# KuldeepChoksi/video-anomaly-detection

Hardware: AMD Instinct MI355X
Metric: frames/sec/GPU (256x256 autoencoder scoring) + AUROC parity vs reference (higher is better)
Workload: dtype f32; 1 GPU; configs[1]: image autoencoder scoring, batch 512 synthetic 256x256x3 frames per GPU; chunk=512, weights=deterministic synthetic state dict (Xavier scale, randomised BN), collective=none (1 GPU)

## Files before the change

include/vad_hip.h:

```cpp
#ifndef VAD_HIP_H
#define VAD_HIP_H
#include <stddef.h>
#ifdef __cplusplus
extern "C" {
#endif

#define VAD_ABI_VERSION 3
#define VAD_OK 0
#define VAD_ERR_ARG (-1)
#define VAD_ERR_HIP (-2)
#define VAD_ERR_WS (-3)

#define VAD_ACT_NONE 0
#define VAD_ACT_LEAKY 1
#define VAD_ACT_RELU 2

#define VAD_PREC_FP32 0
#define VAD_PREC_SPLIT 1
#define VAD_PREC_BF16 2
#define VAD_PREC_BF16S 3
#define VAD_PREC_WINO 4

int vad_abi_version(void);
const char* vad_last_error(void);
// ... 1 lines not shown

size_t vad_pack_conv3x3_floats(int cout, int cin);
int vad_pack_conv3x3(const float* w_oihw, const float* bias, const float* const* bn,
                     int cout, int cin, int precision, float* w_packed, float* bias_out);

size_t vad_pack_conv3x3_c3_floats(int cout);
int vad_pack_conv3x3_c3(const float* w_oihw, const float* bias, const float* const* bn,
                        int cout, float* w_packed, float* bias_out);

size_t vad_pack_convt2x2_floats(int cin, int cout);
int vad_pack_convt2x2(const float* w_iohw, const float* bias, const float* const* bn,
                      int cin, int cout, int precision, float* w_packed, float* bias_out);

size_t vad_pack_conv1x1_floats(int cout, int cin);
int vad_pack_conv1x1(const float* w_oihw, const float* bias, int cout, int cin,
                     float* w_packed, float* bias_out);


int vad_conv3x3_c3(const float* x_nchw, const float* w_packed, const float* bias, float* out_nhwc,
                   int n, int h, int w, int cout, int act, int pool, void* stream);

int vad_conv3x3_c3_fused(const float* x_nchw, const float* w0, const float* b0, const float* w1, const float* b1,
                         float* out_nhwc, int n, int h, int w, int precision, void* stream);

int vad_conv3x3(const float* in_nhwc, long long in_fs, const float* w_packed, const float* bias,
                float* out_nhwc, long long out_fs, int n, int h, int w, int cin, int cout,
                int act, int pool, int precision, void* stream);

size_t vad_pack_conv3x3_wino_floats(int cout, int cin);
int vad_pack_conv3x3_wino(const float* w_oihw, const float* bias, const float* const* bn, int cout, int cin,
                          float* w_packed, float* bias_out);
int vad_conv3x3_wino(const float* in_nhwc, long long in_fs, const float* w_packed, const float* bias,
                     float* out_nhwc, long long out_fs, int n, int h, int w, int cin, int cout,
                     int act, int pool, void* stream);
int vad_convlstm_step_wino(const float* x, long long x_fs, const float* h_prev, long long h_prev_fs, const float* c_prev,
                           const float* w_packed, const float* bias, float* h_out, long long h_out_fs, float* c_out,
                           float* z_ws, int n, int h, int w, int cin_x, int hid, void* stream);

int vad_convt2x2(const float* in_nhwc, long long in_fs, const float* w_packed, const float* bias,
                 float* out_nhwc, long long out_fs, int n, int h, int w, int cin, int cout,
                 int act, int precision, void* stream);

int vad_conv1x1(const float* in_nhwc, const float* w_packed, const float* bias, float* out_nhwc,
                long long npix, int cin, int cout, void* stream);

int vad_convlstm_step(const float* x, long long x_fs, const float* h_prev, long long h_prev_fs,
// ... 240 lines not shown
```

video-anomaly-detection_amd/csrc/conv_mfma.hip:

```cpp
#include <atomic>
#include <type_traits>
#include "vad_common.h"

enum { MODE_PLAIN = 0, MODE_POOL = 1, MODE_LSTM = 2 };

struct Conv3P {
    const float* in;  long long in_fs;  int cin_a;
    const float* in2; long long in2_fs;
    const float* w;   const float* bias;
    float* out;       long long out_fs;
    const float* c_prev; float* c_out;
    const float* zx; long long zx_fs;
    const float* w0; const float* b0;
    int xu8;
    int n, h, w_, cin, cout, hid;
    int tiles_x, tiles_y, cblocks;
    unsigned nblocks;
    unsigned long long* dbg;
    int stagger;
    float* stats;
};

#define MFMA32(a, b, c) __builtin_amdgcn_mfma_f32_32x32x2f32((a), (b), (c), 0, 0, 0)
#define VAD_KORDER(jj) (((jj) == 1) ? 2 : ((jj) == 2) ? 1 : (jj))
// ... 411 lines not shown
        else { if (act == VAD_ACT_LEAKY) GATE_LAUNCH(VAD_ACT_LEAKY, 0) else if (act == VAD_ACT_RELU) GATE_LAUNCH(VAD_ACT_RELU, 0) else GATE_LAUNCH(VAD_ACT_NONE, 0) }
#undef GATE_LAUNCH
        VAD_LAUNCH_CHECK();
        return VAD_OK;
    }
    if (cout % 64 == 0) {
        const long long px = (long long)n * ((wd + 15) / 16);
        const long long nb_thr = cout % 128 == 0 ? px * ((h + 7) / 8) * (cout / 128) : px * ((h + 15) / 16) * (cout / 64);
        if (nb_thr < vad_num_cus() && !with_stats) return pool ? L3(32, 1, 1, 2, 2, MODE_POOL) : L3(32, 1, 1, 2, 2, MODE_PLAIN);
    }
    if (cout % 128 == 0) {
        const long long nb8 = (long long)n * ((wd + 15) / 16) * ((h + 7) / 8) * (cout / 128);
        if (!pool && nb8 < 768) return L3(32, 1, 2, 2, 2, MODE_PLAIN);
        return pool ? L3(32, 2, 2, 2, 2, MODE_POOL) : L3(32, 2, 2, 2, 2, MODE_PLAIN);
    } else if (cout % 64 == 0) {
        if (kn.conv64) return pool ? L3(32, 2, 1, 2, 2, MODE_POOL) : L3(32, 2, 1, 2, 2, MODE_PLAIN);
        return pool ? L3(32, 2, 2, 4, 1, MODE_POOL) : L3(32, 2, 2, 4, 1, MODE_PLAIN);
    } else {
        return pool ? L3(32, 2, 1, 4, 1, MODE_POOL) : L3(32, 2, 1, 4, 1, MODE_PLAIN);
    }
#undef L3
}

extern "C" int vad_conv3x3_c3_fused(const float* x, const float* w0, const float* b0, const float* w1,
                                    const float* b1, float* out, int n, int h, int wd, int precision, void* stream) {
    return vad_conv3x3_c3_fused_fmt(x, VAD_X_F32_NCHW, w0, b0, w1, b1, out, n, h, wd, precision, stream);
}

int vad_conv3x3_c3_fused_fmt(const void* x, int fmt, const float* w0, const float* b0, const float* w1,
                             const float* b1, float* out, int n, int h, int wd, int precision, void* stream) {
    VAD_REQUIRE(x && w0 && b0 && w1 && b1 && out, "conv3x3_c3_fused: null pointer");
    VAD_REQUIRE(precision == VAD_PREC_FP32 || precision == VAD_PREC_SPLIT, "conv3x3_c3_fused: precision=%d must be VAD_PREC_FP32 (0) or VAD_PREC_SPLIT (1)", precision);
    const ConvKnobs kn;
    VAD_REQUIRE(fmt == VAD_X_F32_NCHW || (fmt == VAD_X_U8_NHWC && (kn.variant != 0 || precision == VAD_PREC_SPLIT)),
                "conv3x3_c3_fused: input format %d unsupported (uint8 input needs the persistent kernel)", fmt);
    VAD_REQUIRE(n > 0 && h > 0 && wd > 0 && h % 2 == 0 && wd % 2 == 0, "conv3x3_c3_fused: bad shape %dx%d", h, wd);
    Conv3P p{};
    p.in = (const float*)x; p.in_fs = (long long)3 * h * wd; p.cin_a = 32;
    p.w = w1; p.bias = b1; p.out = out; p.out_fs = (long long)(h / 2) * (wd / 2) * 32;
    p.w0 = w0; p.b0 = b0; p.xu8 = fmt == VAD_X_U8_NHWC;
    p.h = h; p.w_ = wd; p.cin = 32; p.cout = 32; p.hid = 0;
    constexpr int TH = 16;
    p.tiles_x = (wd + 15) / 16; p.tiles_y = (h + TH - 1) / TH; p.cblocks = 1;
    const long long nb = (long long)n * p.tiles_x * p.tiles_y;
    VAD_REQUIRE(nb < (1ll << 31), "conv3x3_c3_fused: grid too large");
    p.nblocks = (unsigned)nb;
    p.n = n;
    if (precision == VAD_PREC_SPLIT) {
        static std::atomic<unsigned> grid_cap1{0};
        unsigned cap = grid_cap1.load(std::memory_order_relaxed);
        if (!cap) grid_cap1 = cap = persistent_grid(conv3x3_mfma_pkernel<32, 2, 1, 4, 1, MODE_POOL, VAD_ACT_LEAKY, 1, 1>, ~0u);
        p.dbg = g_vad_dbg;
        hipLaunchKernelGGL((conv3x3_mfma_pkernel<32, 2, 1, 4, 1, MODE_POOL, VAD_ACT_LEAKY, 1, 1>), dim3(persistent_grid_for(p, cap)), dim3(256), 0,
                           (hipStream_t)stream, p);
    } else if (kn.variant == 0) {
        hipLaunchKernelGGL((conv3x3_mfma_kernel<32, 2, 1, 4, 1, MODE_POOL, VAD_ACT_LEAKY, 1>), dim3((unsigned)nb), dim3(256), 0,
                           (hipStream_t)stream, p);
    } else {
        static std::atomic<unsigned> grid_cap{0};
        unsigned cap = grid_cap.load(std::memory_order_relaxed);
        if (!cap) grid_cap = cap = persistent_grid(conv3x3_mfma_pkernel<32, 2, 1, 4, 1, MODE_POOL, VAD_ACT_LEAKY, 1>, ~0u);
        p.dbg = g_vad_dbg;
        hipLaunchKernelGGL((conv3x3_mfma_pkernel<32, 2, 1, 4, 1, MODE_POOL, VAD_ACT_LEAKY, 1>), dim3(persistent_grid_for(p, cap)), dim3(256), 0,
                           (hipStream_t)stream, p);
    }
    VAD_LAUNCH_CHECK();
    return VAD_OK;
}

bool vad_convlstm_gate_wins(int n, int h, int wd, int hid) { const ConvKnobs kn; return kn.variant != 0 && !kn.no_small && vad_gate_kernel_wins(n, h, wd, hid, kn) != 0; }

bool vad_convlstm_small_wins(int n, int h, int wd, int hid) {
    const long long nb_big = (long long)n * ((wd + 15) / 16) * ((h + 3) / 4) * (hid / 64);
    const int ncu = vad_num_cus();
    const long long m_big = (nb_big + ncu - 1) / ncu;
    const double cost_big = 2.0 * (double)(m_big / 2) + 1.107 * (double)(m_big % 2);
    const double cost_small = 1.178 * (double)nb_big / (double)ncu;
    return nb_big < ncu || cost_small < cost_big;
}

extern "C" int vad_convlstm_step(const float* x, long long x_fs, const float* h_prev, long long h_prev_fs, const float* c_prev,
                                 const float* w, const float* bias, float* h_out, long long h_out_fs,
                                 float* c_out, int n, int h, int wd, int cin_x, int hid, int precision, void* stream) {
    return vad_convlstm_step_zx(x, x_fs, nullptr, 0, h_prev, h_prev_fs, c_prev, w, bias, h_out, h_out_fs, c_out, n, h, wd, cin_x, hid, precision, stream);
}

int vad_convlstm_step_zx(const float* x, long long x_fs, const float* zx, long long zx_fs, const float* h_prev, long long h_prev_fs,
// ... 742 lines not shown
```

video-anomaly-detection_amd/csrc/conv_pkernel.h:

```cpp
#pragma once

__device__ __forceinline__ void pf_set(float& d, float v) { d = v; }
__device__ __forceinline__ void pf_set(float& d, f32x4 v) { d = v[0]; }
__device__ __forceinline__ void pf_set(f32x4& d, f32x4 v) { d = v; }
__device__ __forceinline__ void pf_set(f32x4& d, float v) { d = f32x4{v, v, v, v}; }
__device__ __forceinline__ float pf_get_f(float v) { return v; }
__device__ __forceinline__ float pf_get_f(f32x4 v) { return v[0]; }
__device__ __forceinline__ f32x4 pf_get_v(f32x4 v) { return v; }
__device__ __forceinline__ f32x4 pf_get_v(float v) { return f32x4{v, v, v, v}; }
__device__ __forceinline__ void pf_set(u32x2& d, u32x2 v) { d = v; }
__device__ __forceinline__ void pf_set(u32x2& d, float) {}
__device__ __forceinline__ void pf_set(u32x2& d, f32x4) {}
__device__ __forceinline__ void pf_set(float& d, u32x2) {}
__device__ __forceinline__ void pf_set(f32x4& d, u32x2) {}
__device__ __forceinline__ float pf_get_f(u32x2 v) { return __uint_as_float(v[0]); }
__device__ __forceinline__ f32x4 pf_get_v(u32x2 v) { return f32x4{__uint_as_float(v[0]), __uint_as_float(v[1]), 0.f, 0.f}; }
__device__ __forceinline__ u32x2 pf_get_u(u32x2 v) { return v; }
__device__ __forceinline__ u32x2 pf_get_u(float) { return u32x2{0u, 0u}; }
__device__ __forceinline__ u32x2 pf_get_u(f32x4) { return u32x2{0u, 0u}; }

#ifdef VAD_STAMPS
#define STAMP(k)                                                                                      \
    {                                                                                                 \
        __builtin_amdgcn_sched_barrier(0);                                                            \
// ... 32 lines not shown
__device__ __forceinline__ void vad_mma16(f32x16& acc, f32x16& corr, f16x8 ah, f16x8 al, f16x8 bh, f16x8 bl) {
    if constexpr (PREC == 2) {
        acc = MFMAB16(ah, bh, acc);
    } else {
        acc = MFMA16(ah, bh, acc);
        corr = MFMA16(ah, bl, corr);
        corr = MFMA16(al, bh, corr);
    }
}

template <int PREC>
__device__ __forceinline__ void tile_put_t(float* tile, int pixoff_plus_ch, int ch, float v) {
    if constexpr (PREC) {
        _Float16 hi, lo;
        vad_split_p<PREC>(v, hi, lo);
        _Float16* blk = (_Float16*)&tile[pixoff_plus_ch - ch + (ch >> 3) * 8];
        blk[ch & 7] = hi;
        blk[8 + (ch & 7)] = lo;
    } else {
        tile[pixoff_plus_ch] = v;
    }
}

template <int CK, int MT, int NT, int WM, int WN, int MODE, int ACT, int FUSE_C3 = 0, int PREC = 0, int WITH_STATS = 0, int IO16 = 0>
__global__ __launch_bounds__(256, (FUSE_C3 && !PREC) ? 3 : 2) void conv3x3_mfma_pkernel(Conv3P p) {
    static_assert(WM * WN == 4, "4 waves per work-group");
    static_assert(MODE != MODE_LSTM || NT == 4, "LSTM mode: one N-tile per gate");
    static_assert(!FUSE_C3 || CK == 32, "fused first layer produces exactly one 32-channel chunk");
    static_assert(CK == 32, "staging slots assume 8 channel quads per pixel");
    static_assert(!IO16 || (PREC == 2 && MODE == MODE_PLAIN && !FUSE_C3), "bf16 tensors: bf16 operands, plain convolution");
    constexpr unsigned ES = IO16 ? 2u : 4u;
    constexpr int TH = 2 * MT * WM, LH = TH + 2, LW = 18, PS = CK + 4;
    constexpr int XH = LH + 2, XW = 20, XS = 20;
    constexpr int NPIX = LH * LW, NT0 = (NPIX + 31) / 32;
    constexpr int TOT = FUSE_C3 ? 3 * XH * XW : NPIX * (CK / 4), NPF = (TOT + 255) / 256;
    constexpr int KS = PREC ? 16 : 8;
    constexpr int NS = 9 * (CK / KS);
    constexpr int PB32 = (MODE == MODE_POOL || FUSE_C3) ? 1 : 3;
    constexpr int PB = (PREC == 2) ? 5 : (PREC && NT <= 2) ? 2 : PREC ? 1 : PB32, NB = PB + 1;
    static_assert(NS % 2 == 0 && NS % NB == 0, "fragment ring parity must be the same in every chunk");
    __shared__ __attribute__((aligned(16))) float tile[NPIX * PS];
    __shared__ float xin[FUSE_C3 ? 3 * XH * XS : 1];

    const int tid = threadIdx.x, lane = tid & 63, wave = tid >> 6;
    const int wm = wave / WN, wn = wave % WN;
    const int li = lane & 31, lh = lane >> 5;
    const int prow = (li >> 1) & 1, pcol = 2 * (li >> 2) + (li & 1);

    const unsigned per_frame = (unsigned)(p.tiles_x * p.tiles_y * p.cblocks);
    unsigned L = vad_xcd_remap(blockIdx.x % per_frame, per_frame);
    const int fg = blockIdx.x / per_frame, fgroups = gridDim.x / per_frame;
    const int cb = L % p.cblocks; L /= p.cblocks;
    constexpr bool STATS = WITH_STATS && MODE == MODE_PLAIN && ACT == VAD_ACT_NONE && !FUSE_C3;
    const unsigned stats_row = (unsigned)(blockIdx.x / per_frame) * (unsigned)(p.tiles_x * p.tiles_y) + L;
    float st_s[STATS ? NT : 1], st_q[STATS ? NT : 1];
#pragma unroll
    for (int nt = 0; nt < (STATS ? NT : 1); ++nt) st_s[nt] = st_q[nt] = 0.f;
    const int x0 = (L % p.tiles_x) * 16, y0 = (L / p.tiles_x) * TH;
    const int H = p.h, W = p.w_;

    int abase[MT];
#pragma unroll
    for (int mt = 0; mt < MT; ++mt)
        abase[mt] = ((2 * (wm * MT + mt) + prow) * LW + pcol) * PS + (PREC ? 8 : 4) * lh;

    const int nch_a = p.cin_a / CK;
    const int nch = (p.in2 ? p.cin : p.cin_a) / CK;
    const unsigned wstep = (unsigned)p.cout * (PREC ? 64u : 32u);
    const unsigned wtap = (unsigned)(p.cin / KS) * wstep;
    const __amdgpu_buffer_rsrc_t rw = vad_rsrc(p.w, (p.stagger & 1) ? 0u : 9u * wtap);

    unsigned svo[NPF];
    int slds0;
    const int c4 = tid & 7;
    if (FUSE_C3) {
        slds0 = 0;
#pragma unroll
        for (int i = 0; i < NPF; ++i) {
            const int idx = tid + 256 * i;
            const int lx = idx % XW, t = idx / XW, ly = t % XH, c = t / XH;
            const int gy = y0 - 2 + ly, gx = x0 - 2 + lx;
            const bool ok = idx < TOT && gy >= 0 && gy < H && gx >= 0 && gx < W;
            svo[i] = !ok ? VAD_OOB
                         : p.xu8 ? (unsigned)(__mul24(__mul24(gy, W) + gx, 3) + c)
                                 : (unsigned)(__mul24(c, __mul24(H, W)) + __mul24(gy, W) + gx) * 4u;
        }
    } else {
        const int pix0 = tid >> 3;
        slds0 = pix0 * PS + c4 * 4;
#pragma unroll
        for (int i = 0; i < NPF; ++i) {
            const int pix = pix0 + 32 * i;
            const int ly = pix / LW, lx = pix - ly * LW;
            const int gy = y0 - 1 + ly, gx = x0 - 1 + lx;
            const bool ok = pix < NPIX && gy >= 0 && gy < H && gx >= 0 && gx < W;
            svo[i] = ok ? (unsigned)(__mul24(__mul24(gy, W) + gx, p.cin_a) + c4 * 4) * ES : VAD_OOB;
        }
    }

    typedef typename std::conditional<FUSE_C3 != 0, float, typename std::conditional<IO16 != 0, u32x2, f32x4>::type>::type pf_t;
    pf_t pf[NPF];
    pf_t pf2[IO16 ? NPF : 1];
    float cpv[MODE == MODE_LSTM ? MT : 1][16];

    const unsigned in_bytes = FUSE_C3 ? (unsigned)(3 * H * W) * (p.xu8 ? 1u : 4u) : (unsigned)(H * W) * (unsigned)p.cin_a * ES;
#define ISSUE_TO(PF_, n_, ch_)         \
    {                                                                                                    \
        const char* src_ = ((ch_) < nch_a) ? (const char*)p.in + ((size_t)(n_) * p.in_fs + (ch_) * CK) * ES            \
                                           : (const char*)p.in2 + ((size_t)(n_) * p.in2_fs + ((ch_) - nch_a) * CK) * ES; \
        const unsigned skip_ = (unsigned)(((ch_) < nch_a) ? (ch_) : (ch_) - nch_a) * CK * ES;            \
        const __amdgpu_buffer_rsrc_t r_ = vad_rsrc(src_, in_bytes - skip_);                              \
        _Pragma("unroll") for (int i_ = 0; i_ < NPF; ++i_) {                                             \
            if constexpr (IO16) pf_set(PF_[i_], __builtin_bit_cast(u32x2, vad_bload2(r_, svo[i_], 0)));  \
            else pf_set(PF_[i_], vad_bload4(r_, svo[i_], 0));                                            \
        }                                                                                                \
    }
#define ISSUE(n_, ch_)                                                                                   \
    {                                                                                                    \
        if constexpr (FUSE_C3) {                                                                         \
            if (p.xu8) {    \
                const __amdgpu_buffer_rsrc_t r_ = vad_rsrc((const unsigned char*)p.in + (size_t)(n_) * p.in_fs, in_bytes); \
                _Pragma("unroll") for (int i_ = 0; i_ < NPF; ++i_)                                       \
                    pf_set(pf[i_], __uint_as_float((unsigned)(unsigned char)__builtin_amdgcn_raw_buffer_load_b8(r_, (int)svo[i_], 0, 0))); \
            } else {                                                                                     \
                const __amdgpu_buffer_rsrc_t r_ = vad_rsrc(p.in + (size_t)(n_) * p.in_fs, in_bytes);     \
                _Pragma("unroll") for (int i_ = 0; i_ < NPF; ++i_) pf_set(pf[i_], vad_bload1(r_, svo[i_], 0)); \
            }                                                                                            \
        } else {                                                                                         \
            const char* src_ = ((ch_) < nch_a) ? (const char*)p.in + ((size_t)(n_) * p.in_fs + (ch_) * CK) * ES            \
                                               : (const char*)p.in2 + ((size_t)(n_) * p.in2_fs + ((ch_) - nch_a) * CK) * ES; \
            const unsigned skip_ = (unsigned)(((ch_) < nch_a) ? (ch_) : (ch_) - nch_a) * CK * ES;        \
            const __amdgpu_buffer_rsrc_t r_ = vad_rsrc(src_, in_bytes - skip_);                          \
            _Pragma("unroll") for (int i_ = 0; i_ < NPF; ++i_) {                                         \
                if constexpr (IO16) pf_set(pf[i_], __builtin_bit_cast(u32x2, vad_bload2(r_, svo[i_], 0))); \
                else pf_set(pf[i_], vad_bload4(r_, svo[i_], 0));                                         \
            }                                                                                            \
        }                                                                                                \
    }

#define XWRITE(xb_)                                                                                      \
    {                                                                                                    \
        _Pragma("unroll") for (int i_ = 0; i_ < NPF; ++i_) {                                             \
            const int idx_ = tid + 256 * i_;                                                             \
            const int lx_ = idx_ % XW, t_ = idx_ / XW;                              \
            float xv_ = pf_get_f(pf[i_]);                                                                \
            if (p.xu8) xv_ = svo[i_] == VAD_OOB ? 0.f : vad_norm_u8(__float_as_uint(xv_));               \
            if (idx_ < TOT) (xb_)[t_ * XS + lx_] = xv_;                                                  \
        }                                                                                                \
    }

#ifdef VAD_STAMPS
    unsigned long long st_sum[10] = {0, 0, 0, 0, 0, 0, 0, 0, 0, 0}, st_prev = 0, st_n = 0;
    const unsigned long long st_t0 = __builtin_amdgcn_s_memtime(), st_r0 = __builtin_amdgcn_s_memrealtime();
#endif

    int n = fg;
    if (n >= p.n) return;
    ISSUE(n, 0);
    const bool deep = IO16 && nch >= 2 && (nch & 1) == 0;
    if constexpr (IO16) {
        if (deep) { ISSUE_TO(pf2, n, 1); }
    }
    if constexpr (FUSE_C3) {
        XWRITE(xin);
        if (n + fgroups < p.n) { ISSUE(n + fgroups, 0); }
    }

    f32x4 a[2][MT], b[NB][NT];
    f16x8 ah[PREC ? 1 : 2][MT], al[PREC ? 1 : 2][MT], bh[NB][NT], bl[NB][NT];
    unsigned wl[NT];
// ... 24 lines not shown
        _Pragma("unroll") for (int mt = (m0); mt < (m1); ++mt) {                                  \
            ah[0][mt] = __builtin_bit_cast(f16x8, *(const f32x4*)&tile[abase[mt] + toff_]);       \
            al[0][mt] = __builtin_bit_cast(f16x8, *(const f32x4*)&tile[abase[mt] + toff_ + 4]);   \
        }                                                                                         \
    }
#define LOAD_A(buf, step)                                                                         \
    {                                                                                             \
        const int toff_ = ((((step) / (CK / KS)) / 3) * LW + (((step) / (CK / KS)) % 3)) * PS +   \
                          ((step) % (CK / KS)) * (PREC ? 16 : 8);                                 \
        _Pragma("unroll") for (int mt = 0; mt < MT; ++mt) {                                       \
            if constexpr (PREC) {                                                                 \
                ah[buf][mt] = __builtin_bit_cast(f16x8, *(const f32x4*)&tile[abase[mt] + toff_]); \
                al[buf][mt] = __builtin_bit_cast(f16x8, *(const f32x4*)&tile[abase[mt] + toff_ + 4]); \
            } else a[buf][mt] = *(const f32x4*)&tile[abase[mt] + toff_];                          \
        }                                                                                         \
    }
#pragma unroll
    for (int s0 = 0; s0 < PB; ++s0) LOAD_B(s0, 0, s0);

    float b0w[(FUSE_C3 && !PREC) ? 14 : 1];
    f16x8 b0h[(FUSE_C3 && PREC) ? 2 : 1], b0l[(FUSE_C3 && PREC) ? 2 : 1];
    float bias0 = 0.f;
    bool interior = false;
    if constexpr (FUSE_C3) {
        if constexpr (PREC) {
            const f32x4* ws = (const f32x4*)(p.w0 + 28 * 32);
#pragma unroll
            for (int ks = 0; ks < 2; ++ks) {
                b0h[ks] = __builtin_bit_cast(f16x8, ws[((ks * 32 + li) * 2 + lh) * 2]);
                b0l[ks] = __builtin_bit_cast(f16x8, ws[((ks * 32 + li) * 2 + lh) * 2 + 1]);
            }
        } else {
        }
        bias0 = p.b0[li];
        interior = y0 > 0 && x0 > 0 && y0 + TH < H && x0 + 16 < W;
    }
#pragma unroll
    for (int nt = 0; nt < NT; ++nt) asm volatile("" ::"v"(bv[nt]));
    if constexpr (FUSE_C3) {
        if constexpr (PREC) {
#pragma unroll
            for (int ks = 0; ks < 2; ++ks) { asm volatile("" ::"v"(b0h[ks])); asm volatile("" ::"v"(b0l[ks])); }
        }
        asm volatile("" ::"v"(bias0));
    }

    const bool full_tile = (y0 + TH <= H) && (x0 + 16 <= W);
    const int ech = (MODE == MODE_LSTM) ? p.hid : p.cout;
    const int ow = (MODE == MODE_POOL) ? (W >> 1) : W, oh = (MODE == MODE_POOL) ? (H >> 1) : H;
    const int ey0 = (MODE == MODE_POOL) ? (y0 >> 1) + wm * MT : y0 + 2 * wm * MT;
    const int ex0 = (MODE == MODE_POOL) ? (x0 >> 1) + lh : x0 + 2 * lh;
    const unsigned erow = (unsigned)__mul24(ow, ech) * ES, ecol = (unsigned)ech * ES;
    unsigned eoff[NT];
#pragma unroll
    for (int nt = 0; nt < NT; ++nt) eoff[nt] = (unsigned)(__mul24(__mul24(ey0, ow) + ex0, ech) + cofs[nt]) * ES;
    const unsigned out_bytes = (unsigned)__mul24(oh, ow) * (unsigned)ech * ES;

    while (true) {
        f32x16 acc[MT][NT];
        f32x16 corr[PREC == 1 ? MT : 1][PREC == 1 ? NT : 1];
        if constexpr (PREC == 1) {
#pragma unroll
            for (int mt = 0; mt < MT; ++mt)
#pragma unroll
                for (int nt = 0; nt < NT; ++nt)
#pragma unroll
                    for (int r = 0; r < 16; ++r) corr[mt][nt][r] = 0.f;
        }
        if constexpr (!FUSE_C3) {
#pragma unroll
            for (int mt = 0; mt < MT; ++mt)
#pragma unroll
                for (int nt = 0; nt < NT; ++nt)
#pragma unroll
                    for (int r = 0; r < 16; ++r) acc[mt][nt][r] = bv[nt];
// ... 82 lines not shown
#pragma unroll
                        for (int ks = 0; ks < 2; ++ks) {
                            c0 = MFMA16(gh[ks], b0h[ks], c0);
                            cc = MFMA16(gh[ks], b0l[ks], cc);
                            cc = MFMA16(gl[ks], b0h[ks], cc);
                        }
                        __builtin_amdgcn_s_setprio(0);
                        const int qb = (t * 32 + 4 * lh) * PS + li;
#pragma unroll
                        for (int r = 0; r < 16; ++r) {
                            const int q2 = t * 32 + (r & 3) + 8 * (r >> 2) + 4 * lh;
                            const int ly2 = q2 / LW, lx2 = q2 - ly2 * LW;
                            const bool inside = interior || ((unsigned)(y0 - 1 + ly2) < (unsigned)H && (unsigned)(x0 - 1 + lx2) < (unsigned)W);
                            const float v = vad_act(fmaf(cc[r], 0x1p-11f, c0[r]), VAD_ACT_LEAKY);
                            if (q2 < NPIX) tile_put_t<PREC>(tile, qb + ((r & 3) + 8 * (r >> 2)) * PS, li, inside ? v : 0.f);
                        }
                    }
                } else {
                constexpr int TPW = (NT0 + 3) / 4;
                f32x16 c0[TPW];
                f32x16 bias16;
#pragma unroll
                for (int r = 0; r < 16; ++r) bias16[r] = bias0;
                int abase0[TPW];
#pragma unroll
                for (int u = 0; u < TPW; ++u) {
                    const int q = (wave + 4 * u) * 32 + li, qc = q < NPIX ? q : NPIX - 1;
                    abase0[u] = (qc / LW) * XS + (qc % LW);
                }
#pragma unroll
                for (int h0 = 0; h0 < 14; h0 += 7) {
                    float av[TPW][7];
#pragma unroll
                    for (int u = 0; u < TPW; ++u)
#pragma unroll
                        for (int s0 = 0; s0 < 7; ++s0) {
                            const int k0 = 2 * (h0 + s0), k1 = 2 * (h0 + s0) + 1;
                            const int o0 = ((k0 / 9) * XH + (k0 % 9) / 3) * XS + (k0 % 3);
                            const int o1 = (k1 < 27) ? ((k1 / 9) * XH + (k1 % 9) / 3) * XS + (k1 % 3) : 0;
                            av[u][s0] = xin[abase0[u] + (lh ? o1 : o0)];
                        }
                    __builtin_amdgcn_sched_barrier(0);
                    __builtin_amdgcn_s_setprio(1);
#pragma unroll
                    for (int s0 = 0; s0 < 7; ++s0)
#pragma unroll
                        for (int u = 0; u < TPW; ++u) c0[u] = MFMA32(av[u][s0], b0w[h0 + s0], (h0 + s0 == 0) ? bias16 : c0[u]);
                    __builtin_amdgcn_s_setprio(0);
                    __builtin_amdgcn_sched_barrier(0);
                }
#pragma unroll
                for (int u = 0; u < TPW; ++u) {
                    const int t = wave + 4 * u;
                    if (t < NT0) {
                        const int qb = (t * 32 + 4 * lh) * PS + li;
                        if (interior && t < NT0 - 1) {
#pragma unroll
                            for (int r = 0; r < 16; ++r)
                                tile_put_t<PREC>(tile, qb + ((r & 3) + 8 * (r >> 2)) * PS, li, vad_act(c0[u][r], VAD_ACT_LEAKY));
                        } else {
#pragma unroll
                            for (int r = 0; r < 16; ++r) {
                                const int q2 = t * 32 + (r & 3) + 8 * (r >> 2) + 4 * lh;
                                const int ly2 = q2 / LW, lx2 = q2 - ly2 * LW;
                                const bool inside = (unsigned)(y0 - 1 + ly2) < (unsigned)H && (unsigned)(x0 - 1 + lx2) < (unsigned)W;
                                const float v = vad_act(c0[u][r], VAD_ACT_LEAKY);
                                if (q2 < NPIX) tile_put_t<PREC>(tile, qb + ((r & 3) + 8 * (r >> 2)) * PS, li, inside ? v : 0.f);
                            }
                        }
                    }
                }
                }
                STAMP(8);
                __syncthreads();
                STAMP(9);
                if (has_next) { XWRITE(xin); }
                if (nn + fgroups < p.n) { ISSUE(nn + fgroups, 0); }
#pragma unroll
                for (int mt = 0; mt < MT; ++mt)
#pragma unroll
                    for (int nt = 0; nt < NT; ++nt)
#pragma unroll
                        for (int r = 0; r < 16; ++r) acc[mt][nt][r] = bv[nt];
            } else {
#pragma unroll
                for (int i = 0; i < NPF; ++i)
                    if ((tid >> 3) + 32 * i < NPIX) {
                        if constexpr (IO16) {
                            float* blk = &tile[(tid >> 3) * PS + i * 32 * PS + (c4 >> 1) * 8 + (c4 & 1) * 2];
                            *(u32x2*)blk = pf_get_u(pf[i]);
                        } else if constexpr (PREC) {
                            const f32x4 v = pf_get_v(pf[i]);
                            float* blk = &tile[(tid >> 3) * PS + i * 32 * PS + (c4 >> 1) * 8 + (c4 & 1) * 2];
                            if constexpr (PREC == 2) {
                                typedef __bf16 bf16x2_t __attribute__((ext_vector_type(2)));
                                typedef unsigned u32x2_t __attribute__((ext_vector_type(2)));
                                const bf16x2_t p0 = {(__bf16)v[0], (__bf16)v[1]}, p1 = {(__bf16)v[2], (__bf16)v[3]};
                                *(u32x2_t*)blk = u32x2_t{__builtin_bit_cast(unsigned, p0), __builtin_bit_cast(unsigned, p1)};
                            } else {
                                f16x4 hi, lo;
#pragma unroll
                                for (int e = 0; e < 4; ++e) { _Float16 h_, l_; vad_split_p<PREC>(v[e], h_, l_); hi[e] = h_; lo[e] = l_; }
                                *(f16x4*)blk = hi;
                                *(f16x4*)(blk + 4) = lo;
                            }
                        } else {
// ... 80 lines not shown
#pragma unroll
            for (int s0 = 0; s0 < PB; ++s0) LOAD_B(s0, 0, s0);
        }

        if (MODE == MODE_LSTM) {
            const __amdgpu_buffer_rsrc_t rc_out = vad_rsrc(p.c_out + (size_t)n * (out_bytes / 4), out_bytes);
            const __amdgpu_buffer_rsrc_t rh_out = vad_rsrc(p.out + (size_t)n * p.out_fs, out_bytes);
#pragma unroll
            for (int mt = 0; mt < MT; ++mt) {
#pragma unroll
                for (int r = 0; r < 16; ++r) {
                    const int dy = 2 * mt + ((r & 3) >> 1), dx = 4 * (r >> 2) + (r & 1);
                    const bool ok = full_tile || ((ey0 + dy) < oh && (ex0 + dx) < ow);
                    const unsigned vo = ok ? eoff[0] : VAD_OOB;
                    const unsigned so = dy * erow + dx * ecol;
                    float cn, hn;
                    vad_lstm_cell(acc[mt][0][r], acc[mt][1][r], acc[mt][2][r], acc[mt][3][r], cpv[mt][r], cn, hn);
                    vad_bstore1(cn, rc_out, vo, so);
                    vad_bstore1(hn, rh_out, vo, so);
                }
            }
        } else {
            const __amdgpu_buffer_rsrc_t ro = vad_rsrc((const char*)p.out + (size_t)n * p.out_fs * ES, (p.stagger & 2) ? 0u : out_bytes);
            if (MODE == MODE_POOL) {
#pragma unroll
                for (int mt = 0; mt < MT; ++mt) {
#pragma unroll
                    for (int q = 0; q < 4; ++q) {
                        const bool ok = full_tile || ((ey0 + mt) < oh && (ex0 + 2 * q) < ow);
                        const unsigned so = mt * erow + 2 * q * ecol;
#pragma unroll
                        for (int nt = 0; nt < NT; ++nt) {
                            const float m = fmaxf(fmaxf(acc[mt][nt][4 * q], acc[mt][nt][4 * q + 1]), fmaxf(acc[mt][nt][4 * q + 2], acc[mt][nt][4 * q + 3]));
                            vad_bstore1(vad_act(m, ACT), ro, ok ? eoff[nt] : VAD_OOB, so);
                        }
                    }
                }
            } else {
                float ts[STATS ? NT : 1], tq[STATS ? NT : 1];
#pragma unroll
                for (int nt = 0; nt < (STATS ? NT : 1); ++nt) ts[nt] = tq[nt] = 0.f;
#pragma unroll
                for (int mt = 0; mt < MT; ++mt) {
#pragma unroll
                    for (int q = 0; q < 4; ++q) {
#pragma unroll
                        for (int pos = 0; pos < 4; ++pos) {
                            const int dy = 2 * mt + (pos >> 1), dx = 4 * q + (pos & 1);
                            const bool ok = full_tile || ((ey0 + dy) < oh && (ex0 + dx) < ow);
                            const unsigned so = dy * erow + dx * ecol;
#pragma unroll
                            for (int nt = 0; nt < NT; ++nt) {
// ... 63 lines not shown
```

video-anomaly-detection_amd/hip.py:

```python
from __future__ import annotations

import ctypes as C
import os
import subprocess
import threading
from pathlib import Path

PKG_DIR = Path(__file__).resolve().parent
REPO_DIR = PKG_DIR.parent
CSRC = PKG_DIR / "csrc"
LIB_PATH = Path(os.environ.get("VAD_LIB", PKG_DIR / "libvad_hip.so"))
SOURCES = ["conv_mfma.hip", "conv_wino.hip", "dec4_fused.hip", "tail.hip", "wide_io.hip", "state_io.hip", "resize_u8.hip", "ssim.hip", "train_ops.hip", "train_step.hip", "train_step_img.hip", "vad_api.hip", "pack.cpp"]

VAD_OK = 0
ABI_VERSION = 3
MAX_IN_CHANNELS = 32
PREC_FP32, PREC_SPLIT, PREC_BF16, PREC_BF16S, PREC_WINO = 0, 1, 2, 3, 4
PRECISIONS = {"fp32": PREC_FP32, "split": PREC_SPLIT, "bf16": PREC_BF16S, "bf16_operands": PREC_BF16, "bf16_tensors": PREC_BF16S,
              "winograd": PREC_WINO}


def training_precision(name: str, trainer: str, tensors: bool) -> str:
    ok = ("fp32", "split", "bf16_operands", "winograd") + (("bf16", "bf16_tensors") if tensors else ())
    if name in ("bf16", "bf16_tensors") and not tensors:
# ... 58 lines not shown

_f32p = C.POINTER(C.c_float)
_vp = C.c_void_p
_ll = C.c_longlong
_i = C.c_int
_sz = C.c_size_t
_f = C.c_float

SIGNATURES = {
    "vad_abi_version": (_i, []),
    "vad_last_error": (C.c_char_p, []),
    "vad_pack_conv3x3_floats": (_sz, [_i, _i]),
    "vad_pack_conv3x3": (_i, [_vp, _vp, _vp, _i, _i, _i, _vp, _vp]),
    "vad_pack_conv3x3_c3_floats": (_sz, [_i]),
    "vad_pack_conv3x3_c3": (_i, [_vp, _vp, _vp, _i, _vp, _vp]),
    "vad_pack_convt2x2_floats": (_sz, [_i, _i]),
    "vad_pack_convt2x2": (_i, [_vp, _vp, _vp, _i, _i, _i, _vp, _vp]),
    "vad_pack_conv1x1_floats": (_sz, [_i, _i]),
    "vad_pack_conv1x1": (_i, [_vp, _vp, _i, _i, _vp, _vp]),
    "vad_pack_conv3x3_to3_floats": (_sz, [_i]),
    "vad_pack_conv3x3_to3": (_i, [_vp, _i, _vp]),
    "vad_conv3x3_c3": (_i, [_vp, _vp, _vp, _vp, _i, _i, _i, _i, _i, _i, _vp]),
    "vad_conv3x3_c3_fused": (_i, [_vp, _vp, _vp, _vp, _vp, _vp, _i, _i, _i, _i, _vp]),
    "vad_conv3x3": (_i, [_vp, _ll, _vp, _vp, _vp, _ll, _i, _i, _i, _i, _i, _i, _i, _i, _vp]),
    "vad_convt2x2": (_i, [_vp, _ll, _vp, _vp, _vp, _ll, _i, _i, _i, _i, _i, _i, _i, _vp]),
    "vad_pack_conv3x3_wino_floats": (_sz, [_i, _i]),
    "vad_pack_conv3x3_wino": (_i, [_vp, _vp, _vp, _i, _i, _vp, _vp]),
    "vad_conv3x3_wino": (_i, [_vp, _ll, _vp, _vp, _vp, _ll, _i, _i, _i, _i, _i, _i, _i, _vp]),
    "vad_convlstm_step_wino": (_i, [_vp, _ll, _vp, _ll, _vp, _vp, _vp, _vp, _ll, _vp, _vp, _i, _i, _i, _i, _i, _vp]),
    "vad_conv1x1": (_i, [_vp, _vp, _vp, _vp, _ll, _i, _i, _vp]),
    "vad_convlstm_step": (_i, [_vp, _ll, _vp, _ll, _vp, _vp, _vp, _vp, _ll, _vp, _i, _i, _i, _i, _i, _i, _vp]),
    "vad_score_partials": (_i, [_i, _i, _i]),
    "vad_conv3x3_to3_score": (_i, [_vp, _vp, _vp, _vp, _vp, _vp, _vp, _i, _i, _i, _i, _vp]),
    "vad_convt2x2_to3_score": (_i, [_vp, _vp, _vp, _vp, _vp, _vp, _vp, _i, _i, _i, _i, _i, _i, _vp]),
    "vad_score_finalize": (_i, [_vp, _i, _i, _i, _i, _vp, _vp, _i, _vp]),
    "vad_nhwc_to_nchw": (_i, [_vp, _vp, _i, _i, _i, _i, _vp]),
    "vad_nchw_to_nhwc": (_i, [_vp, _vp, _i, _i, _i, _i, _vp]),
    "vad_ssim_workspace_floats": (_sz, [_ll, _i, _i]),
    "vad_ssim_mse": (_i, [_vp, _vp, _ll, _i, _i, _i, C.c_float, _vp, _vp, _vp]),
    "vad_ssim_grad_workspace_floats": (_sz, [_ll, _i, _i]),
    "vad_ssim_mse_backward": (_i, [_vp, _vp, _ll, _i, _i, _i, C.c_float, _vp, _vp, _vp, _vp]),
    "vad_chan_ws_floats": (_sz, [_ll, _i]),
    "vad_bn_stats": (_i, [_vp, _ll, _i, _f, _f, _vp, _vp, _vp, _vp, _vp]),
    "vad_chan_sum": (_i, [_vp, _ll, _i, _vp, _vp, _vp]),
    "vad_bn_act_pool_fwd": (_i, [_vp, _vp, _vp, _vp, _vp, _ll, _i, _i, _i, _i, _i, _i, _i, _i, _i, _vp]),
    "vad_bn_act_pool_bwd": (_i, [_vp, _vp, _vp, _vp, _vp, _ll, _i, _i, _i, _vp, _i, _vp, _vp, _vp, _vp,
# ... 195 lines not shown
```

Measured before the change: 17150 frames/s.

## Specialize fused first-layer persistent kernel on uint8 input and simplify halo handling

Adds a compile-time XU8 template parameter so the fused first conv layer branches on uint8-versus-float input at compile time instead of at runtime. In the fp32 path, per-element boundary checks on the layer-0 tile writes are replaced by a separate pass that zeroes only the out-of-image halo rows and columns of edge tiles. It also precomputes LDS address bases per tap delta, and adds a branch-free pooling epilogue for full tiles. This aims to cut ALU and branch overhead in the first layer, at the cost of an extra barrier on edge tiles and more kernel instantiations.

```diff
diff --git a/include/vad_hip.h b/include/vad_hip.h
--- a/include/vad_hip.h
+++ b/include/vad_hip.h
@@ -47,6 +47,8 @@
 
 int vad_conv3x3_c3_fused(const float* x_nchw, const float* w0, const float* b0, const float* w1, const float* b1,
                          float* out_nhwc, int n, int h, int w, int precision, void* stream);
+int vad_conv3x3_c3_fused_x(const void* x, int x_format, const float* w0, const float* b0, const float* w1, const float* b1,
+                           float* out_nhwc, int n, int h, int w, int precision, void* stream);
 
 int vad_conv3x3(const float* in_nhwc, long long in_fs, const float* w_packed, const float* bias,
                 float* out_nhwc, long long out_fs, int n, int h, int w, int cin, int cout,
diff --git a/video-anomaly-detection_amd/csrc/conv_mfma.hip b/video-anomaly-detection_amd/csrc/conv_mfma.hip
--- a/video-anomaly-detection_amd/csrc/conv_mfma.hip
+++ b/video-anomaly-detection_amd/csrc/conv_mfma.hip
@@ -457,9 +457,23 @@
 #undef L3
 }
 
+template <int PREC, int XU8>
+static void launch_c3_fused_persistent(Conv3P& p, hipStream_t s) {
+    static std::atomic<unsigned> grid_cap{0};
+    unsigned cap = grid_cap.load(std::memory_order_relaxed);
+    if (!cap) grid_cap = cap = persistent_grid(conv3x3_mfma_pkernel<32, 2, 1, 4, 1, MODE_POOL, VAD_ACT_LEAKY, 1, PREC, 0, 0, XU8>, ~0u);
+    p.dbg = g_vad_dbg;
+    hipLaunchKernelGGL((conv3x3_mfma_pkernel<32, 2, 1, 4, 1, MODE_POOL, VAD_ACT_LEAKY, 1, PREC, 0, 0, XU8>), dim3(persistent_grid_for(p, cap)), dim3(256), 0, s, p);
+}
+
 extern "C" int vad_conv3x3_c3_fused(const float* x, const float* w0, const float* b0, const float* w1,
                                     const float* b1, float* out, int n, int h, int wd, int precision, void* stream) {
     return vad_conv3x3_c3_fused_fmt(x, VAD_X_F32_NCHW, w0, b0, w1, b1, out, n, h, wd, precision, stream);
+}
+
+extern "C" int vad_conv3x3_c3_fused_x(const void* x, int x_format, const float* w0, const float* b0, const float* w1,
+                                      const float* b1, float* out, int n, int h, int wd, int precision, void* stream) {
+    return vad_conv3x3_c3_fused_fmt(x, x_format, w0, b0, w1, b1, out, n, h, wd, precision, stream);
 }
 
 int vad_conv3x3_c3_fused_fmt(const void* x, int fmt, const float* w0, const float* b0, const float* w1,
@@ -482,22 +496,14 @@
     p.nblocks = (unsigned)nb;
     p.n = n;
     if (precision == VAD_PREC_SPLIT) {
-        static std::atomic<unsigned> grid_cap1{0};
-        unsigned cap = grid_cap1.load(std::memory_order_relaxed);
-        if (!cap) grid_cap1 = cap = persistent_grid(conv3x3_mfma_pkernel<32, 2, 1, 4, 1, MODE_POOL, VAD_ACT_LEAKY, 1, 1>, ~0u);
-        p.dbg = g_vad_dbg;
-        hipLaunchKernelGGL((conv3x3_mfma_pkernel<32, 2, 1, 4, 1, MODE_POOL, VAD_ACT_LEAKY, 1, 1>), dim3(persistent_grid_for(p, cap)), dim3(256), 0,
-                           (hipStream_t)stream, p);
+        if (p.xu8) launch_c3_fused_persistent<1, 1>(p, (hipStream_t)stream);
+        else launch_c3_fused_persistent<1, 0>(p, (hipStream_t)stream);
     } else if (kn.variant == 0) {
         hipLaunchKernelGGL((conv3x3_mfma_kernel<32, 2, 1, 4, 1, MODE_POOL, VAD_ACT_LEAKY, 1>), dim3((unsigned)nb), dim3(256), 0,
                            (hipStream_t)stream, p);
     } else {
-        static std::atomic<unsigned> grid_cap{0};
-        unsigned cap = grid_cap.load(std::memory_order_relaxed);
-        if (!cap) grid_cap = cap = persistent_grid(conv3x3_mfma_pkernel<32, 2, 1, 4, 1, MODE_POOL, VAD_ACT_LEAKY, 1>, ~0u);
-        p.dbg = g_vad_dbg;
-        hipLaunchKernelGGL((conv3x3_mfma_pkernel<32, 2, 1, 4, 1, MODE_POOL, VAD_ACT_LEAKY, 1>), dim3(persistent_grid_for(p, cap)), dim3(256), 0,
-                           (hipStream_t)stream, p);
+        if (p.xu8) launch_c3_fused_persistent<0, 1>(p, (hipStream_t)stream);
+        else launch_c3_fused_persistent<0, 0>(p, (hipStream_t)stream);
     }
     VAD_LAUNCH_CHECK();
     return VAD_OK;
diff --git a/video-anomaly-detection_amd/csrc/conv_pkernel.h b/video-anomaly-detection_amd/csrc/conv_pkernel.h
--- a/video-anomaly-detection_amd/csrc/conv_pkernel.h
+++ b/video-anomaly-detection_amd/csrc/conv_pkernel.h
@@ -78,13 +78,14 @@
     }
 }
 
-template <int CK, int MT, int NT, int WM, int WN, int MODE, int ACT, int FUSE_C3 = 0, int PREC = 0, int WITH_STATS = 0, int IO16 = 0>
+template <int CK, int MT, int NT, int WM, int WN, int MODE, int ACT, int FUSE_C3 = 0, int PREC = 0, int WITH_STATS = 0, int IO16 = 0, int XU8 = 0>
 __global__ __launch_bounds__(256, (FUSE_C3 && !PREC) ? 3 : 2) void conv3x3_mfma_pkernel(Conv3P p) {
     static_assert(WM * WN == 4, "4 waves per work-group");
     static_assert(MODE != MODE_LSTM || NT == 4, "LSTM mode: one N-tile per gate");
     static_assert(!FUSE_C3 || CK == 32, "fused first layer produces exactly one 32-channel chunk");
     static_assert(CK == 32, "staging slots assume 8 channel quads per pixel");
     static_assert(!IO16 || (PREC == 2 && MODE == MODE_PLAIN && !FUSE_C3), "bf16 tensors: bf16 operands, plain convolution");
+    static_assert(!XU8 || FUSE_C3, "uint8 frames enter through the fused first layer only");
     constexpr unsigned ES = IO16 ? 2u : 4u;
     constexpr int TH = 2 * MT * WM, LH = TH + 2, LW = 18, PS = CK + 4;
     constexpr int XH = LH + 2, XW = 20, XS = 20;
@@ -120,15 +121,16 @@
     for (int mt = 0; mt < MT; ++mt)
         abase[mt] = ((2 * (wm * MT + mt) + prow) * LW + pcol) * PS + (PREC ? 8 : 4) * lh;
 
-    const int nch_a = p.cin_a / CK;
-    const int nch = (p.in2 ? p.cin : p.cin_a) / CK;
-    const unsigned wstep = (unsigned)p.cout * (PREC ? 64u : 32u);
-    const unsigned wtap = (unsigned)(p.cin / KS) * wstep;
+    const int nch_a = FUSE_C3 ? 1 : p.cin_a / CK;
+    const int nch = FUSE_C3 ? 1 : (p.in2 ? p.cin : p.cin_a) / CK;
+    const unsigned wstep = (unsigned)(FUSE_C3 ? 32 : p.cout) * (PREC ? 64u : 32u);
+    const unsigned wtap = (unsigned)((FUSE_C3 ? 32 : p.cin) / KS) * wstep;
     const __amdgpu_buffer_rsrc_t rw = vad_rsrc(p.w, (p.stagger & 1) ? 0u : 9u * wtap);
 
     unsigned svo[NPF];
     int slds0;
     const int c4 = tid & 7;
+    unsigned xpad = 0;
     if (FUSE_C3) {
         slds0 = 0;
 #pragma unroll
@@ -138,8 +140,9 @@
             const int gy = y0 - 2 + ly, gx = x0 - 2 + lx;
             const bool ok = idx < TOT && gy >= 0 && gy < H && gx >= 0 && gx < W;
             svo[i] = !ok ? VAD_OOB
-                         : p.xu8 ? (unsigned)(__mul24(__mul24(gy, W) + gx, 3) + c)
-                                 : (unsigned)(__mul24(c, __mul24(H, W)) + __mul24(gy, W) + gx) * 4u;
+                         : XU8 ? (unsigned)(__mul24(__mul24(gy, W) + gx, 3) + c)
+                               : (unsigned)(__mul24(c, __mul24(H, W)) + __mul24(gy, W) + gx) * 4u;
+            if (XU8 && !ok) xpad |= 1u << i;
         }
     } else {
         const int pix0 = tid >> 3;
@@ -159,7 +162,7 @@
     pf_t pf2[IO16 ? NPF : 1];
     float cpv[MODE == MODE_LSTM ? MT : 1][16];
 
-    const unsigned in_bytes = FUSE_C3 ? (unsigned)(3 * H * W) * (p.xu8 ? 1u : 4u) : (unsigned)(H * W) * (unsigned)p.cin_a * ES;
+    const unsigned in_bytes = FUSE_C3 ? (unsigned)(3 * H * W) * (XU8 ? 1u : 4u) : (unsigned)(H * W) * (unsigned)p.cin_a * ES;
 #define ISSUE_TO(PF_, n_, ch_)         \
     {                                                                                                    \
         const char* src_ = ((ch_) < nch_a) ? (const char*)p.in + ((size_t)(n_) * p.in_fs + (ch_) * CK) * ES            \
@@ -174,7 +177,7 @@
 #define ISSUE(n_, ch_)                                                                                   \
     {                                                                                                    \
         if constexpr (FUSE_C3) {                                                                         \
-            if (p.xu8) {    \
+            if constexpr (XU8) {    \
                 const __amdgpu_buffer_rsrc_t r_ = vad_rsrc((const unsigned char*)p.in + (size_t)(n_) * p.in_fs, in_bytes); \
                 _Pragma("unroll") for (int i_ = 0; i_ < NPF; ++i_)                                       \
                     pf_set(pf[i_], __uint_as_float((unsigned)(unsigned char)__builtin_amdgcn_raw_buffer_load_b8(r_, (int)svo[i_], 0, 0))); \
@@ -194,14 +197,16 @@
         }                                                                                                \
     }
 
+    static_assert(XS == XW, "halo buffer rows are dense: staging slot = LDS float index");
 #define XWRITE(xb_)                                                                                      \
     {                                                                                                    \
+        unsigned xp_ = xpad;    \
+        if constexpr (XU8) asm volatile("" : "+v"(xp_));                                                 \
         _Pragma("unroll") for (int i_ = 0; i_ < NPF; ++i_) {                                             \
-            const int idx_ = tid + 256 * i_;                                                             \
-            const int lx_ = idx_ % XW, t_ = idx_ / XW;                              \
             float xv_ = pf_get_f(pf[i_]);                                                                \
-            if (p.xu8) xv_ = svo[i_] == VAD_OOB ? 0.f : vad_norm_u8(__float_as_uint(xv_));               \
-            if (idx_ < TOT) (xb_)[t_ * XS + lx_] = xv_;                                                  \
+            if constexpr (XU8)    \
+                xv_ = __uint_as_float(__float_as_uint(vad_norm_u8(__float_as_uint(xv_))) & ~(unsigned)__builtin_amdgcn_sbfe((int)xp_, i_, 1)); \
+            if (256 * (i_ + 1) <= TOT || tid < TOT - 256 * i_) (xb_)[tid + 256 * i_] = xv_;              \
         }                                                                                                \
     }
 
@@ -272,6 +277,7 @@
     f16x8 b0h[(FUSE_C3 && PREC) ? 2 : 1], b0l[(FUSE_C3 && PREC) ? 2 : 1];
     float bias0 = 0.f;
     bool interior = false;
+    int zline[4] = {-1, -1, -1, -1};
     if constexpr (FUSE_C3) {
         if constexpr (PREC) {
             const f32x4* ws = (const f32x4*)(p.w0 + 28 * 32);
@@ -284,6 +290,12 @@
         }
         bias0 = p.b0[li];
         interior = y0 > 0 && x0 > 0 && y0 + TH < H && x0 + 16 < W;
+        if constexpr (!PREC) {
+            zline[0] = y0 == 0 ? 0 : -1;
+            zline[1] = H - y0 + 1 < LH ? H - y0 + 1 : -1;
+            zline[2] = x0 == 0 ? 0 : -1;
+            zline[3] = W - x0 + 1 < LW ? W - x0 + 1 : -1;
+        }
     }
 #pragma unroll
     for (int nt = 0; nt < NT; ++nt) asm volatile("" ::"v"(bv[nt]));
@@ -300,7 +312,7 @@
     const int ow = (MODE == MODE_POOL) ? (W >> 1) : W, oh = (MODE == MODE_POOL) ? (H >> 1) : H;
     const int ey0 = (MODE == MODE_POOL) ? (y0 >> 1) + wm * MT : y0 + 2 * wm * MT;
     const int ex0 = (MODE == MODE_POOL) ? (x0 >> 1) + lh : x0 + 2 * lh;
-    const unsigned erow = (unsigned)__mul24(ow, ech) * ES, ecol = (unsigned)ech * ES;
+    const unsigned erow = (unsigned)__mul24(ow, ech) * ES, ecol = FUSE_C3 ? 32u * ES : (unsigned)ech * ES;
     unsigned eoff[NT];
 #pragma unroll
     for (int nt = 0; nt < NT; ++nt) eoff[nt] = (unsigned)(__mul24(__mul24(ey0, ow) + ex0, ech) + cofs[nt]) * ES;
@@ -429,11 +441,16 @@
                 f32x16 bias16;
 #pragma unroll
                 for (int r = 0; r < 16; ++r) bias16[r] = bias0;
-                int abase0[TPW];
+                constexpr int D_ROW = XS - 2, D_PLANE = (XH - 2) * XS - 2;
+                int abase0[TPW][4];
 #pragma unroll
                 for (int u = 0; u < TPW; ++u) {
                     const int q = (wave + 4 * u) * 32 + li, qc = q < NPIX ? q : NPIX - 1;
-                    abase0[u] = (qc / LW) * XS + (qc % LW);
+                    const int ab = (qc / LW) * XS + (qc % LW);
+                    abase0[u][0] = ab + lh;
+                    abase0[u][1] = ab + lh * D_ROW;
+                    abase0[u][2] = ab + lh * D_PLANE;
+                    abase0[u][3] = lh ? ab : ab + (2 * XH + 2) * XS + 2;
                 }
 #pragma unroll
                 for (int h0 = 0; h0 < 14; h0 += 7) {
@@ -445,7 +462,9 @@
                             const int k0 = 2 * (h0 + s0), k1 = 2 * (h0 + s0) + 1;
                             const int o0 = ((k0 / 9) * XH + (k0 % 9) / 3) * XS + (k0 % 3);
                             const int o1 = (k1 < 27) ? ((k1 / 9) * XH + (k1 % 9) / 3) * XS + (k1 % 3) : 0;
-                            av[u][s0] = xin[abase0[u] + (lh ? o1 : o0)];
+                            const int d = o1 - o0;
+                            if (k1 >= 27) av[u][s0] = xin[abase0[u][3]];
+                            else av[u][s0] = xin[abase0[u][d == 1 ? 0 : d == D_ROW ? 1 : 2] + o0];
                         }
                     __builtin_amdgcn_sched_barrier(0);
                     __builtin_amdgcn_s_setprio(1);
@@ -456,24 +475,26 @@
                     __builtin_amdgcn_s_setprio(0);
                     __builtin_amdgcn_sched_barrier(0);
                 }
+                constexpr int REM = NPIX - 32 * (NT0 - 1);
+                const int wv = __builtin_amdgcn_readfirstlane(wave);
 #pragma unroll
                 for (int u = 0; u < TPW; ++u) {
-                    const int t = wave + 4 * u;
-                    if (t < NT0) {
-                        const int qb = (t * 32 + 4 * lh) * PS + li;
-                        if (interior && t < NT0 - 1) {
+                    const int t = wv + 4 * u;
+                    const int qb = (t * 32 + 4 * lh) * PS + li;
+                    if (4 * u + 3 < NT0 - 1 || t < NT0 - 1) {
+#pragma unroll
+                        for (int r = 0; r < 16; ++r)
+                            tile_put_t<PREC>(tile, qb + ((r & 3) + 8 * (r >> 2)) * PS, li, vad_act(c0[u][r], VAD_ACT_LEAKY));
+                    } else if (4 * u + 3 >= NT0 - 1 && t == NT0 - 1) {
+#pragma unroll
+                        for (int r = 0; r < 16; ++r)
+                            if ((r & 3) + 8 * (r >> 2) + 4 < REM)
+                                tile_put_t<PREC>(tile, qb + ((r & 3) + 8 * (r >> 2)) * PS, li, vad_act(c0[u][r], VAD_ACT_LEAKY));
+                        if (lh == 0) {
 #pragma unroll
                             for (int r = 0; r < 16; ++r)
-                                tile_put_t<PREC>(tile, qb + ((r & 3) + 8 * (r >> 2)) * PS, li, vad_act(c0[u][r], VAD_ACT_LEAKY));
-                        } else {
-#pragma unroll
-                            for (int r = 0; r < 16; ++r) {
-                                const int q2 = t * 32 + (r & 3) + 8 * (r >> 2) + 4 * lh;
-                                const int ly2 = q2 / LW, lx2 = q2 - ly2 * LW;
-                                const bool inside = (unsigned)(y0 - 1 + ly2) < (unsigned)H && (unsigned)(x0 - 1 + lx2) < (unsigned)W;
-                                const float v = vad_act(c0[u][r], VAD_ACT_LEAKY);
-                                if (q2 < NPIX) tile_put_t<PREC>(tile, qb + ((r & 3) + 8 * (r >> 2)) * PS, li, inside ? v : 0.f);
-                            }
+                                if ((r & 3) + 8 * (r >> 2) < REM && (r & 3) + 8 * (r >> 2) + 4 >= REM)
+                                    tile_put_t<PREC>(tile, qb + ((r & 3) + 8 * (r >> 2)) * PS, li, vad_act(c0[u][r], VAD_ACT_LEAKY));
                         }
                     }
                 }
@@ -481,6 +502,21 @@
                 STAMP(8);
                 __syncthreads();
                 STAMP(9);
+                if constexpr (!PREC) {
+                    static_assert(LH == LW, "zeroing slots assume a square halo tile");
+                    if (!interior) {
+                        int zt = tid;
+                        asm volatile("" : "+v"(zt));
+#pragma unroll
+                        for (int i = 0; i < (4 * LW * 8 + 255) / 256; ++i) {
+                            const int idx = zt + 256 * i;
+                            const int seg = idx / (LW * 8), rem = idx - seg * (LW * 8), pix = rem >> 3;
+                            const int line = seg == 0 ? zline[0] : seg == 1 ? zline[1] : seg == 2 ? zline[2] : zline[3];
+                            const int q = seg < 2 ? line * LW + pix : pix * LW + line;
+                            if (idx < 4 * LW * 8 && line >= 0) *(f32x4*)&tile[q * PS + (rem & 7) * 4] = f32x4{0.f, 0.f, 0.f, 0.f};
+                        }
+                    }
+                }
                 if (has_next) { XWRITE(xin); }
                 if (nn + fgroups < p.n) { ISSUE(nn + fgroups, 0); }
 #pragma unroll
@@ -489,6 +525,9 @@
                     for (int nt = 0; nt < NT; ++nt)
 #pragma unroll
                         for (int r = 0; r < 16; ++r) acc[mt][nt][r] = bv[nt];
+                if constexpr (!PREC) {
+                    if (!interior) __syncthreads();
+                }
             } else {
 #pragma unroll
                 for (int i = 0; i < NPF; ++i)
@@ -615,12 +654,33 @@
             }
         } else {
             const __amdgpu_buffer_rsrc_t ro = vad_rsrc((const char*)p.out + (size_t)n * p.out_fs * ES, (p.stagger & 2) ? 0u : out_bytes);
-            if (MODE == MODE_POOL) {
+            constexpr bool EPI_BRANCH = FUSE_C3 && !PREC;
+            static_assert(!EPI_BRANCH || MODE == MODE_POOL, "the fused first layer ends in the pooling epilogue");
+            auto epi_origin = [&](int& ey, int& ex) {
+                int t_ = tid;
+                asm volatile("" : "+v"(t_));
+                const int wm_ = (t_ >> 6) / WN, lh_ = (t_ >> 5) & 1;
+                ey = (y0 >> 1) + wm_ * MT;
+                ex = (x0 >> 1) + lh_;
+            };
+            if (EPI_BRANCH && MODE == MODE_POOL && full_tile) {
+#pragma unroll
+                for (int mt = 0; mt < MT; ++mt)
+#pragma unroll
+                    for (int q = 0; q < 4; ++q)
+#pragma unroll
+                        for (int nt = 0; nt < NT; ++nt) {
+                            const float m = fmaxf(fmaxf(acc[mt][nt][4 * q], acc[mt][nt][4 * q + 1]), fmaxf(acc[mt][nt][4 * q + 2], acc[mt][nt][4 * q + 3]));
+                            vad_bstore1(vad_act(m, ACT), ro, eoff[nt], mt * erow + 2 * q * ecol);
+                        }
+            } else if (MODE == MODE_POOL) {
+                int ey0_ = ey0, ex0_ = ex0;
+                if constexpr (EPI_BRANCH) epi_origin(ey0_, ex0_);
 #pragma unroll
                 for (int mt = 0; mt < MT; ++mt) {
 #pragma unroll
                     for (int q = 0; q < 4; ++q) {
-                        const bool ok = full_tile || ((ey0 + mt) < oh && (ex0 + 2 * q) < ow);
+                        const bool ok = (!EPI_BRANCH && full_tile) || ((ey0_ + mt) < oh && (ex0_ + 2 * q) < ow);
                         const unsigned so = mt * erow + 2 * q * ecol;
 #pragma unroll
                         for (int nt = 0; nt < NT; ++nt) {
diff --git a/video-anomaly-detection_amd/hip.py b/video-anomaly-detection_amd/hip.py
--- a/video-anomaly-detection_amd/hip.py
+++ b/video-anomaly-detection_amd/hip.py
@@ -104,6 +104,7 @@
     "vad_pack_conv3x3_to3": (_i, [_vp, _i, _vp]),
     "vad_conv3x3_c3": (_i, [_vp, _vp, _vp, _vp, _i, _i, _i, _i, _i, _i, _vp]),
     "vad_conv3x3_c3_fused": (_i, [_vp, _vp, _vp, _vp, _vp, _vp, _i, _i, _i, _i, _vp]),
+    "vad_conv3x3_c3_fused_x": (_i, [_vp, _i, _vp, _vp, _vp, _vp, _vp, _i, _i, _i, _i, _vp]),
     "vad_conv3x3": (_i, [_vp, _ll, _vp, _vp, _vp, _ll, _i, _i, _i, _i, _i, _i, _i, _i, _vp]),
     "vad_convt2x2": (_i, [_vp, _ll, _vp, _vp, _vp, _ll, _i, _i, _i, _i, _i, _i, _i, _vp]),
     "vad_pack_conv3x3_wino_floats": (_sz, [_i, _i]),
```

New measurement: 17340 frames/s (median of 6 runs). 1.01x the previous value.
